# zrjer/Sparse-Matrix-Factorization-Library

Hardware: AMD Instinct MI355X
Metric: numeric-factorization GFLOP/s (supernodal Cholesky) (higher is better)
Workload: dtype f64; 1 GPU; 3D 7-point Laplacian 128^3 SPD Cholesky fp64, geometric ND, devSlotSize 8694792192; n=2097152, nnz_input=8339456, nsuper=35419, factor_doubles=3787034536, parallelism=single GPU, grid_rule=BASELINE config

## Files before the change

sparse-matrix-factorization-library_amd/csrc/sf_kernels.hip:

```cpp
#include "sf_kernels.h"
#include <cstdlib>
#include "sf_wave.h"

namespace sf {

typedef double double4_t __attribute__((ext_vector_type(4)));
typedef double double2_t __attribute__((ext_vector_type(2), aligned(8)));

__device__ __forceinline__ int lower_bound_i32(const int32_t* __restrict__ a, int n, int32_t key) {
    int lo = 0, hi = n;
    while (lo < hi) {
        const int mid = (lo + hi) >> 1;
        if (a[mid] < key) lo = mid + 1; else hi = mid;
    }
    return lo;
}

__global__ void __launch_bounds__(256)
k_load_panels(const int64_t* __restrict__ Lp, const int32_t* __restrict__ Li, const double* __restrict__ Lx, int32_t n,
              const int32_t* __restrict__ Super, const int32_t* __restrict__ SuperMap,
              const int64_t* __restrict__ Lsip, const int32_t* __restrict__ Lsi,
              const int64_t* __restrict__ Lsxp, double* __restrict__ Lsx, int skip_diag,
              const int8_t* __restrict__ load_mask) {
    const int32_t j = blockIdx.x * blockDim.x + threadIdx.x;
// ... 137 lines not shown
    return __hiloint2double(__builtin_amdgcn_readlane(__double2hiint(v), l), __builtin_amdgcn_readlane(__double2loint(v), l));
}

template <bool RCP, int W>
__device__ __forceinline__ void getrf_panel_wave(double (&a)[W], int lane, int J0, int b, double tol, double eps, bool& bad, int& nperturbed,
                                                 int& pos, bool& active, int* piv_rows) {
#pragma unroll
    for (int j = 0; j < W; ++j) {
        const int J = J0 + j;
        int p = J;
        if (tol > 0.0 && J < b) {
            const double nat = readlane_dyn_f64(a[j], J);
            const unsigned long long act = __ballot(active);
            const bool nat_free = ((act >> J) & 1ull) != 0;
            const double anat = fabs(nat);
            const unsigned long long larger = __ballot(active && !(tol * fabs(a[j]) <= anat));
            if (!(nat_free && larger == 0ull && nat != 0.0)) {
                double m;
                const int pm = wave_argmax_abs(a[j], active, &m);
                if (!(nat_free && fabs(nat) >= tol * m && nat != 0.0) && pm >= 0) p = pm;
            }
            p = __builtin_amdgcn_readfirstlane(p);
        }
        double piv = readlane_dyn_f64(a[j], p);
        if (J < b && eps > 0.0 && !(fabs(piv) >= eps) && piv == piv) {
            piv = (piv < 0.0) ? -eps : eps;
            ++nperturbed;
            if (lane == p) a[j] = piv;
        }
        bad = bad || !(piv != 0.0);
        const bool elim = active && lane != p;
        double l;
        if (RCP) {
            const double rp = rcp_full(piv);
            l = elim ? a[j] * rp : 0.0;
        } else {
            l = elim ? a[j] / piv : 0.0;
        }
        if (elim) a[j] = l;
        if (lane == p) { pos = J; active = false; }
        if (piv_rows != nullptr && lane == 0) piv_rows[J] = p;
#pragma unroll
        for (int c = j + 1; c < W; ++c) a[c] -= l * readlane_dyn_f64(a[c], p);
    }
}

template <int W>
__device__ __forceinline__ bool getrf_panel_natural(double (&a)[W], int lane, int J0, int b, double tol, double eps) {
    unsigned long long viol = 0ull;
#pragma unroll
    for (int j = 0; j < W; ++j) {
        const int J = J0 + j;
        const double piv = readlane_dyn_f64(a[j], J);
        const bool below = lane > J;
        viol |= __ballot(below && !(tol * fabs(a[j]) <= fabs(piv)));
        if (J < b && (!(fabs(piv) >= eps) || piv == 0.0)) viol |= 1ull;
        const double rp = rcp_full(piv);
        const double l = below ? a[j] * rp : 0.0;
        if (below) a[j] = l;
#pragma unroll
        for (int c = j + 1; c < W; ++c) a[c] -= l * readlane_dyn_f64(a[c], J);
    }
    return viol == 0ull;
}

template <int W>
__device__ __forceinline__ void getrf_block_w(const PotrfTask& t, double* __restrict__ Lsx, int64_t u_shift, int* __restrict__ info, const PivotCtl& pc) {
    double* PLd = Lsx + t.panel + t.diag + (int64_t)t.diag * t.ld;
    double* PUd = PLd + u_shift;
    const int b = t.b;
    const int lane = threadIdx.x;
    const int64_t ld = t.ld;

    double a[W];
#pragma unroll
    for (int c = 0; c < W; ++c) {
        double v = (c == lane) ? 1.0 : 0.0;
        if (lane < b && c < b) v = (c < lane) ? PLd[lane + c * ld] : PUd[c + lane * ld];
        a[c] = v;
    }
    bool bad = false, active = lane < b;
    int np = 0, pos = lane;
    getrf_panel_wave<false, W>(a, lane, 0, b, pc.tol, pc.eps, bad, np, pos, active, nullptr);
    if (bad && lane == 0) atomicOr(info, 1);
    if (np > 0 && lane == 0) atomicAdd(pc.nperturb, np);
#pragma unroll
    for (int c = 0; c < W; ++c) {
        if (lane < b && c < b) {
            if (c < pos) PLd[pos + c * ld] = a[c]; else PUd[c + pos * ld] = a[c];
        }
    }
    if (pc.pivpos && lane < b) {
        const int g0 = t.first_col + t.diag;
        pc.pivpos[g0 + lane] = g0 + pos;
        pc.pivinv[g0 + pos] = g0 + lane;
    }
}

__global__ void __launch_bounds__(64)
k_getrf_block(const PotrfTask* __restrict__ tasks, double* __restrict__ Lsx, int64_t u_shift, int* __restrict__ info, PivotCtl pc) {
    const PotrfTask t = tasks[blockIdx.x];
    if (t.b <= 8) getrf_block_w<8>(t, Lsx, u_shift, info, pc);
    else if (t.b <= 16) getrf_block_w<16>(t, Lsx, u_shift, info, pc);
    else if (t.b <= 32) getrf_block_w<32>(t, Lsx, u_shift, info, pc);
    else getrf_block_w<NB>(t, Lsx, u_shift, info, pc);
}

void launch_getrf(const PotrfTask* tasks, int ntasks, double* Lsx, int64_t u_shift, int* info, PivotCtl pc, hipStream_t st) {
    if (ntasks <= 0) return;
    hipLaunchKernelGGL(k_getrf_block, dim3(ntasks), dim3(64), 0, st, tasks, Lsx, u_shift, info, pc);
}

__global__ void __launch_bounds__(256)
k_pack_lu(const int32_t* __restrict__ Super, const int64_t* __restrict__ Lsip, const int64_t* __restrict__ Xp,
          const int64_t* __restrict__ RefXp, int32_t nsuper, const double* __restrict__ PL, const double* __restrict__ PU,
          double* __restrict__ out, int64_t e_begin, int64_t e_end) {
    for (int64_t e = e_begin + (int64_t)blockIdx.x * blockDim.x + threadIdx.x; e < e_end; e += (int64_t)gridDim.x * blockDim.x) {
        double* __restrict__ dst = out + (e - e_begin);
        int lo = 0, hi = nsuper;
        while (hi - lo > 1) {
            const int mid = (lo + hi) >> 1;
            if (RefXp[mid] <= e) lo = mid; else hi = mid;
        }
        const int s = lo;
        if (Xp[s] < 0) { *dst = 0.0; continue; }
        const int64_t nscol = Super[s + 1] - Super[s], nsrow = Lsip[s + 1] - Lsip[s];
        const int64_t lda = 2 * nsrow - nscol;
        const int64_t off = e - RefXp[s];
        const int64_t j = off / lda, R = off % lda;
        const double* pl = PL + Xp[s] + j * nsrow;
        double v;
        if (R < nscol) v = (R > j) ? pl[R] : PU[Xp[s] + j + R * nsrow];
        else if (R < nsrow) v = pl[R];
        else v = PU[Xp[s] + (R - nsrow + nscol) + j * nsrow];
        *dst = v;
    }
}

void launch_pack_lu(const int32_t* Super, const int64_t* Lsip, const int64_t* Xp, const int64_t* RefXp, int32_t nsuper,
                    const double* PL, const double* PU, double* out, int64_t e_begin, int64_t e_end, hipStream_t st) {
    if (e_end <= e_begin) return;
    const int64_t blocks = (e_end - e_begin + 255) / 256;
    hipLaunchKernelGGL(k_pack_lu, dim3((unsigned)(blocks < 65536 ? blocks : 65536)), dim3(256), 0, st,
                       Super, Lsip, Xp, RefXp, nsuper, PL, PU, out, e_begin, e_end);
}

__global__ void __launch_bounds__(256)
k_factor_hash(const int32_t* __restrict__ Super, const int64_t* __restrict__ Lsip, const int64_t* __restrict__ Xp,
              const int64_t* __restrict__ RefXp, int32_t nsuper, const double* __restrict__ PL, const double* __restrict__ PU, int lu,
              int64_t total, int64_t chunk, unsigned long long* __restrict__ H) {
    const int64_t begin = (int64_t)blockIdx.x * chunk, end = min(begin + chunk, total);
    if (begin >= end) return;
    const bool idle = begin + threadIdx.x >= end;
    int64_t e = idle ? end - 1 : begin + threadIdx.x;
    int lo = 0, hi = nsuper;
    while (hi - lo > 1) {
        const int mid = (lo + hi) >> 1;
        if (RefXp[mid] <= e) lo = mid; else hi = mid;
    }
    int s = lo;
    unsigned long long acc = 0;
    int64_t s_end = RefXp[s + 1], s_beg = RefXp[s], xp = Xp[s];
    int64_t nscol = Super[s + 1] - Super[s], nsrow = Lsip[s + 1] - Lsip[s];
    if (idle) e = end;
    for (; e < end; e += 256) {
        if (e >= s_end) {
            if (acc) atomicAdd(&H[s], acc);
            acc = 0;
            while (e >= RefXp[s + 1]) ++s;
            s_end = RefXp[s + 1]; s_beg = RefXp[s]; xp = Xp[s];
            nscol = Super[s + 1] - Super[s]; nsrow = Lsip[s + 1] - Lsip[s];
        }
        if (xp < 0) {
            e += ((s_end - e + 255) / 256 - 1) * 256;
            continue;
        }
        const int64_t off = e - s_beg;
        double v;
        if (!lu) {
            v = PL[xp + off];
        } else {
            const int64_t lda = 2 * nsrow - nscol;
            const int64_t j = off / lda, R = off % lda;
            if (R < nscol) v = (R > j) ? PL[xp + j * nsrow + R] : PU[xp + j + R * nsrow];
            else if (R < nsrow) v = PL[xp + j * nsrow + R];
            else v = PU[xp + (R - nsrow + nscol) + j * nsrow];
        }
        acc += (unsigned long long)__double_as_longlong(v) * ((2ull * (unsigned long long)e + 1ull) * 0x9E3779B97F4A7C15ull);
    }
    __shared__ int s_first;
    __shared__ unsigned long long s_part[4];
    if (threadIdx.x == 0) s_first = s;
    __syncthreads();
    const bool uniform = __syncthreads_and(s == s_first) != 0;
    if (!uniform) { if (acc) atomicAdd(&H[s], acc); return; }
    for (int off = 32; off > 0; off >>= 1) acc += __shfl_down(acc, off, 64);
    if ((threadIdx.x & 63) == 0) s_part[threadIdx.x >> 6] = acc;
    __syncthreads();
    if (threadIdx.x == 0) {
        const unsigned long long tot = s_part[0] + s_part[1] + s_part[2] + s_part[3];
        if (tot) atomicAdd(&H[s], tot);
    }
}

void launch_factor_hash(const int32_t* Super, const int64_t* Lsip, const int64_t* Xp, const int64_t* RefXp, int32_t nsuper,
                        const double* PL, const double* PU, int lu, int64_t total, unsigned long long* H, hipStream_t st) {
    if (total <= 0 || nsuper <= 0) return;
    const int64_t chunk = 256 * 64;
    const int64_t blocks = (total + chunk - 1) / chunk;
    hipLaunchKernelGGL(k_factor_hash, dim3((unsigned)blocks), dim3(256), 0, st, Super, Lsip, Xp, RefXp, nsuper, PL, PU, lu, total, chunk, H);
}

__global__ void __launch_bounds__(256)
k_lu_fill_u11(const FillTile* __restrict__ tiles, double* __restrict__ PL, const double* __restrict__ PU) {
    __shared__ double tile[64][65];
    const FillTile t = tiles[blockIdx.x];
    const int tx = threadIdx.x & 63, ty = threadIdx.x >> 6;
    const int jlo = max(t.c0, t.cb), jhi = min(t.c0 + 64, t.ce);
    {
        const int j = t.c0 + tx;
        for (int rr = ty; rr < 64; rr += 4) {
            const int R = t.r0 + rr;
            if (j >= jlo && j < jhi && R <= j) tile[rr][tx] = PU[t.xp + j + (int64_t)R * t.nsrow];
        }
    }
    __syncthreads();
    {
        const int R = t.r0 + tx;
        for (int jj = ty; jj < 64; jj += 4) {
            const int j = t.c0 + jj;
            if (j >= jlo && j < jhi && R <= j) PL[t.xp + R + (int64_t)j * t.nsrow] = tile[tx][jj];
        }
    }
}

void launch_lu_fill_u11(const FillTile* tiles, int64_t ntiles, double* PL, const double* PU, hipStream_t st) {
    if (ntiles <= 0) return;
    hipLaunchKernelGGL(k_lu_fill_u11, dim3((unsigned)ntiles), dim3(256), 0, st, tiles, PL, PU);
}

__global__ void __launch_bounds__(TRSM_ROWS)
k_trsm_block(const TrsmTask* __restrict__ tasks, double* __restrict__ Lsx, const int32_t* __restrict__ pivinv) {
    __shared__ __attribute__((aligned(16))) double Dt[NB][NB];
    __shared__ double Dinv[NB];
    const TrsmTask t = tasks[blockIdx.x];
    const double* Dg = Lsx + t.dpanel + t.diag + (int64_t)t.diag * t.ld;
    const int b = t.b;
    const int tid = threadIdx.x;

    for (int e = tid; e < b * NB; e += (int)blockDim.x) {
        const int k = e / NB, j = e % NB;
        Dt[k][j] = (j < b && k < j) ? Dg[j + (int64_t)k * t.ld] : 0.0;
    }
    if (tid < NB) Dinv[tid] = (tid < b && !t.unit) ? 1.0 / Dg[tid + (int64_t)tid * t.ld] : 1.0;
    __syncthreads();

    if (tid >= t.nrows) return;
    double* X = Lsx + t.panel + t.row0 + tid + (int64_t)t.diag * t.ld;
    const int64_t ld = t.ld;
    if (pivinv && t.unit) {
        const int g0 = t.first_col + t.diag;
        const int32_t* pv = pivinv + g0;
        double tmp[NB];
#pragma unroll
        for (int c = 0; c < NB; ++c) tmp[c] = X[(int64_t)(pv[min(c, b - 1)] - g0) * ld];
#pragma unroll
        for (int c = 0; c < NB; ++c)
            if (c < b) X[(int64_t)c * ld] = tmp[c];
    }

    for (int jb = 0; jb < b; jb += 8) {
        double acc[8];
#pragma unroll
        for (int u = 0; u < 8; ++u) acc[u] = X[min(jb + u, b - 1) * ld];
#pragma unroll
        for (int u = 0; u < 8; ++u) acc[u] = (jb + u < b) ? acc[u] : 0.0;
        for (int k0 = 0; k0 < jb; k0 += 8) {
            double xk[8];
#pragma unroll
            for (int v = 0; v < 8; ++v) xk[v] = X[(k0 + v) * ld];
#pragma unroll
            for (int v = 0; v < 8; ++v)
#pragma unroll
                for (int u = 0; u < 8; ++u) acc[u] -= xk[v] * Dt[k0 + v][jb + u];
        }
#pragma unroll
        for (int u = 0; u < 8; ++u) {
#pragma unroll
            for (int v = 0; v < u; ++v) acc[u] -= acc[v] * Dt[jb + v][jb + u];
            acc[u] *= Dinv[jb + u];
        }
#pragma unroll
        for (int u = 0; u < 8; ++u)
            if (jb + u < b) X[(jb + u) * ld] = acc[u];
    }
}

void launch_trsm(const TrsmTask* tasks, int ntasks, double* Lsx, const int32_t* pivinv, hipStream_t st) {
    if (ntasks <= 0) return;
    hipLaunchKernelGGL(k_trsm_block, dim3(ntasks), dim3(TRSM_ROWS), 0, st, tasks, Lsx, pivinv);
}

constexpr int LDS_LD = GEMM_BM + 16;

__device__ __forceinline__ int last_le_u32(const uint32_t* __restrict__ a, int n, uint32_t key) {
    int lo = 0, hi = n;
    while (hi - lo > 1) {
        const int mid = (lo + hi) >> 1;
        if (a[mid] <= key) lo = mid; else hi = mid;
    }
    return lo;
}

__device__ double g_zero_page[GEMM_BM + 16];

__device__ __forceinline__ void glds16(const void* gsrc, uint32_t lds_dst) {
    unsigned keep;
    asm volatile("s_mov_b32 %0, m0\n\ts_mov_b32 m0, %2\n\ts_nop 0\n\tglobal_load_lds_dwordx4 %1, off\n\ts_mov_b32 m0, %0"
                 : "=&s"(keep) : "v"(gsrc), "s"(lds_dst) : "memory");
}
__device__ __forceinline__ uint32_t lds_addr(const void* p) {
    return __builtin_amdgcn_readfirstlane((uint32_t)(uintptr_t)(__attribute__((address_space(3))) const void*)p);
}

#ifdef SF_EXP_TIMING
__device__ unsigned long long* g_exp_stamps = nullptr;
void exp_set_stamps(unsigned long long* p) { (void)hipMemcpyToSymbol(HIP_SYMBOL(g_exp_stamps), &p, sizeof(p)); }
#define SF_STAMP(slot) do { if (tid == 0 && g_exp_stamps && exp_tile < 64) \
        g_exp_stamps[((size_t)blockIdx.x * 64 + exp_tile) * 4 + (slot)] = __builtin_amdgcn_s_memtime(); } while (0)
#else
#define SF_STAMP(slot) do { } while (0)
#endif

template <int MODE, bool DMA>
__global__ void __launch_bounds__(GEMM_THREADS, GEMM_WAVES / 2)
k_gemm(const GemmProb* __restrict__ probs, const GemmTask* __restrict__ tasks,
       const uint32_t* __restrict__ kt_prefix, int ntasks, uint32_t u_lo, uint32_t u_hi,
       double* __restrict__ Lsx, const int32_t* __restrict__ RelMap, int* __restrict__ ticket, int whole_tiles, uint32_t min_units) {
    __shared__ int s_claim;
    __shared__ __attribute__((aligned(16))) double Ys[2][GEMM_BK][LDS_LD];
    __shared__ __attribute__((aligned(16))) double Xs[2][GEMM_BK][LDS_LD];
    __shared__ int32_t rowmap[GEMM_BM];
    __shared__ int32_t colmap[GEMM_BN];

    constexpr int WCJ = GEMM_BN / (GEMM_WAVES / 2);
    constexpr int TMN = WCJ / 16;
    constexpr int SQ = GEMM_BK / GEMM_WAVES;
    const int tid = threadIdx.x;
    const int lane = tid & 63, wave = tid >> 6;
    const int wm = wave & 1, wn = wave >> 1;
    const int fr = lane & 15, fk = lane >> 4;

    const uint32_t T = u_hi - u_lo;
    const uint32_t G = gridDim.x;
    const uint32_t xcd = blockIdx.x & 7;
    const uint32_t xcd_n = (G >> 3) + (xcd < (G & 7) ? 1u : 0u);
    const uint32_t xcd_base = xcd < (G & 7) ? xcd * ((G >> 3) + 1) : (G & 7) * ((G >> 3) + 1) + (xcd - (G & 7)) * (G >> 3);
    const uint32_t share = xcd_base + (blockIdx.x >> 3);
    (void)T;
    int t0 = last_le_u32(kt_prefix, ntasks + 1, u_lo);
    if (kt_prefix[t0] < u_lo) ++t0;
    const int t1 = last_le_u32(kt_prefix, ntasks + 1, u_hi);
    const int R = (t1 > t0) ? (int)(((uint32_t)(t1 - t0) + (whole_tiles ? G - 1 : 0)) / G) : 0;
    const uint32_t head_end = (R > 0) ? kt_prefix[t0] : u_hi;
    const uint32_t tail_beg = (R > 0 && !whole_tiles) ? kt_prefix[t0 + R * (int)G] : u_hi;

    int ph = 0, rr = 0;
#ifdef SF_EXP_DEPHASE
    bool exp_dephased = false;
#endif
#ifdef SF_EXP_TIMING
    int exp_tile = 0;
    if (tid == 0 && g_exp_stamps) {
        g_exp_stamps[(size_t)gridDim.x * 256 + blockIdx.x * 4 + 0] = __builtin_amdgcn_s_memtime();
        g_exp_stamps[(size_t)gridDim.x * 256 + blockIdx.x * 4 + 1] = wall_clock64();
    }
#endif
    for (;;) {
    uint32_t u, u_end;
    int ti;
    SF_STAMP(0);
    if (ph == 1) {
        uint32_t slot = share;
        if (ticket != nullptr && R > 0) {
            if (tid == 0) s_claim = __hip_atomic_fetch_add(ticket + xcd, 1, __ATOMIC_RELAXED, __HIP_MEMORY_SCOPE_AGENT);
            __syncthreads();
            const uint32_t c = (uint32_t)__builtin_amdgcn_readfirstlane(s_claim);
            rr = (int)(c / xcd_n);
            slot = xcd_base + c % xcd_n;
        }
        if (rr >= R) { ph = 2; continue; }
        ti = t0 + rr * (int)G + (int)slot;
        ++rr;
        if (ti >= t1) continue;
        u = kt_prefix[ti];
        u_end = kt_prefix[ti + 1];
#ifdef SF_EXP_DEPHASE
        if (!exp_dephased && blockIdx.x >= gridDim.x / 2) {
            const int naps = (int)(u_end - u) * SF_EXP_DEPHASE / 16;
            for (int i = 0; i < naps; ++i) __builtin_amdgcn_s_sleep(127);
        }
        exp_dephased = true;
#endif
    } else {
        const uint32_t ra = (ph == 0) ? u_lo : tail_beg, rb = (ph == 0) ? head_end : u_hi;
        const uint32_t Ueq = (rb > ra) ? (rb - ra + G - 1) / G : 0, U = max(Ueq, min_units);
        const uint32_t sh = (U > Ueq) ? blockIdx.x : share;
        if (rb <= ra || sh * U >= rb - ra) {
            if (ph == 0) { ph = 1; continue; }
            break;
        }
        u = ra + sh * U;
        u_end = min(rb, u + U);
        ti = last_le_u32(kt_prefix, ntasks + 1, u);
    }

    while (u < u_end) {
        const GemmTask tk = tasks[ti];
        const GemmProb pb = probs[tk.prob];
        const uint32_t tbase = kt_prefix[ti];
        const int nkt = (int)(kt_prefix[ti + 1] - tbase);
        const int kt0 = (int)(u - tbase);
        const int kt1 = min(nkt, kt0 + (int)(u_end - u));
        u += (uint32_t)(kt1 - kt0);
        ++ti;

        const int ci0 = tk.tm * GEMM_BM, cj0 = tk.tn * GEMM_BN;
        const int M = pb.M, N = pb.N;
        const int lda = pb.lda;
        const int kfirst = (int)tk.kt0 * GEMM_BK;
        const int K = min(pb.K - kfirst, nkt * GEMM_BK);
        const double* __restrict__ Yg = Lsx + pb.y_off + ci0 + (int64_t)kfirst * lda;
        const double* __restrict__ Xg = Lsx + pb.x_off + cj0 + (int64_t)kfirst * lda;

        if (MODE == 1) {
            if (tid < GEMM_BM) {
                const int ci = ci0 + tid;
                rowmap[tid] = (ci < M) ? RelMap[pb.map_off + ci] : 0;
            } else if (tid < GEMM_BM + GEMM_BN) {
                const int cj = cj0 + (tid - GEMM_BM);
                colmap[tid - GEMM_BM] = (cj < N) ? RelMap[pb.map_off + cj] : 0;
            }
        }

        const int prow = 2 * (tid & 63), pk0 = tid >> 6;
        const bool y0_ok = (ci0 + prow) < M, y1_ok = (ci0 + prow + 1) < M;
        const bool x0_ok = (cj0 + prow) < N, x1_ok = (cj0 + prow + 1) < N;
        const double* __restrict__ yp = Yg + (y0_ok ? prow : 0);
        const double* __restrict__ xp = Xg + (x0_ok ? prow : 0);
        double2_t ry[DMA ? 1 : SQ], rx[DMA ? 1 : SQ];

        auto load_tile = [&](int k0) {
            if (DMA) return;
#pragma unroll
            for (int q = 0; q < SQ; ++q) {
                const int64_t off = (int64_t)min(k0 + pk0 + GEMM_WAVES * q, K - 1) * lda;
                ry[q] = *reinterpret_cast<const double2_t*>(yp + off);
                rx[q] = *reinterpret_cast<const double2_t*>(xp + off);
            }
        };
        auto store_tile = [&](int buf, int k0) {
            if (DMA) {
#pragma unroll
                for (int q = 0; q < SQ; ++q) {
                    const int kl = pk0 + GEMM_WAVES * q, k = k0 + kl;
                    const bool kin = k < K;
                    const double* ysrc = yp + (int64_t)min(k, K - 1) * lda;
                    const double* xsrc = kin ? xp + (int64_t)k * lda : g_zero_page + prow;
                    glds16(ysrc, lds_addr(&Ys[buf][kl][0]));
                    glds16(xsrc, lds_addr(&Xs[buf][kl][0]));
                }
                return;
            }
#pragma unroll
            for (int q = 0; q < SQ; ++q) {
                const bool kin = (k0 + pk0 + GEMM_WAVES * q) < K;
                double2_t vy = ry[q], vx = rx[q];
                vy.x = (kin && y0_ok) ? vy.x : 0.0; vy.y = (kin && y1_ok) ? vy.y : 0.0;
                vx.x = (kin && x0_ok) ? vx.x : 0.0; vx.y = (kin && x1_ok) ? vx.y : 0.0;
                *reinterpret_cast<double2_t*>(&Ys[buf][pk0 + GEMM_WAVES * q][prow]) = vy;
                *reinterpret_cast<double2_t*>(&Xs[buf][pk0 + GEMM_WAVES * q][prow]) = vx;
            }
        };

        const int qci0 = ci0 + wm * 64, qcj0 = cj0 + wn * WCJ;
        const bool quad_active = __builtin_amdgcn_readfirstlane((int)((qci0 < M) && (qcj0 < N) && (qci0 + 63 >= qcj0))) != 0;

        double4_t acc[TMN][4];
#pragma unroll
        for (int a = 0; a < TMN; ++a)
#pragma unroll
            for (int b = 0; b < 4; ++b) acc[a][b] = (double4_t){0.0, 0.0, 0.0, 0.0};

        load_tile(kt0 * GEMM_BK);
        store_tile(0, kt0 * GEMM_BK);
        if (DMA) asm volatile("s_waitcnt vmcnt(0)" ::: "memory");
        __syncthreads();
        SF_STAMP(1);
        load_tile((kt0 + 1) * GEMM_BK);
        int buf = 0;
        if (quad_active) {
            for (int kt = kt0; kt < kt1; ++kt) {
#pragma unroll
                for (int kk = 0; kk < GEMM_BK / 4; ++kk) {
                    double a[TMN], b[4];
#pragma unroll
                    for (int t = 0; t < TMN; ++t) a[t] = Xs[buf][kk * 4 + fk][wn * WCJ + t * 16 + fr];
#pragma unroll
                    for (int t = 0; t < 4; ++t) b[t] = Ys[buf][kk * 4 + fk][wm * 64 + t * 16 + fr];
                    if (kk == 0) store_tile(buf ^ 1, (kt + 1) * GEMM_BK);
                    if (kk == 1) load_tile((kt + 2) * GEMM_BK);
#pragma unroll
                    for (int tm = 0; tm < TMN; ++tm)
#pragma unroll
                        for (int tn = 0; tn < 4; ++tn)
                            acc[tm][tn] = __builtin_amdgcn_mfma_f64_16x16x4f64(a[tm], b[tn], acc[tm][tn], 0, 0, 0);
                }
                if (DMA) asm volatile("s_waitcnt vmcnt(0)" ::: "memory");
                __syncthreads();
                buf ^= 1;
            }
        } else {
            for (int kt = kt0; kt < kt1; ++kt) {
                store_tile(buf ^ 1, (kt + 1) * GEMM_BK);
                load_tile((kt + 2) * GEMM_BK);
                if (DMA) asm volatile("s_waitcnt vmcnt(0)" ::: "memory");
                __syncthreads();
                buf ^= 1;
            }
        }

        SF_STAMP(2);
#ifdef SF_EXP_SKIP_EPILOGUE
        if (quad_active) {
            double v = 0.0;
            for (int tm = 0; tm < TMN; ++tm) for (int tn = 0; tn < 4; ++tn) for (int r = 0; r < 4; ++r) v += acc[tm][tn][r];
            if (v == 12345.678) Lsx[pb.c_off] = v;
        }
#else
        if (quad_active) {
            double* __restrict__ Cg = Lsx + pb.c_off;
            const int64_t ldc = pb.ldc;
#pragma unroll
            for (int tm = 0; tm < TMN; ++tm) {
#pragma unroll
                for (int tn = 0; tn < 4; ++tn) {
                    const int lci = wm * 64 + tn * 16 + fr;
                    const int ci = ci0 + lci;
#pragma unroll
                    for (int r = 0; r < 4; ++r) {
                        const int lcj = wn * WCJ + tm * 16 + fk + 4 * r;
                        const int cj = cj0 + lcj;
                        if (ci < M && cj < N && ci >= cj + (pb.strict & 1)) {
                            const double v = acc[tm][tn][r];
                            if (MODE == 1) {
                                unsafeAtomicAdd(Cg + rowmap[lci] + (int64_t)colmap[lcj] * ldc, -v);
                            } else {
                                double* dst = Cg + ci + (int64_t)cj * ldc;
                                unsafeAtomicAdd(dst, -v);
                            }
                        }
                    }
                }
            }
        }
#endif
        __syncthreads();
        SF_STAMP(3);
#ifdef SF_EXP_TIMING
        ++exp_tile;
        SF_STAMP(0);
#endif
    }
    if (ph == 2) break;
    if (ph == 0) ph = 1;
    }
#ifdef SF_EXP_TIMING
    if (tid == 0 && g_exp_stamps) {
        g_exp_stamps[(size_t)gridDim.x * 256 + blockIdx.x * 4 + 2] = __builtin_amdgcn_s_memtime();
        g_exp_stamps[(size_t)gridDim.x * 256 + blockIdx.x * 4 + 3] = wall_clock64();
    }
#endif
}

#ifndef SF_LU_STEP_WGS
#define SF_LU_STEP_WGS 3
#endif
#ifndef SF_GEMM_MIN_UNITS_DEFAULT
#define SF_GEMM_MIN_UNITS_DEFAULT 16
#endif
#ifndef SF_POTRF_PW
#define SF_POTRF_PW 16
#endif
constexpr int ST_ULD = ST_ROWS + 1;
constexpr int ST_KC = 32;
constexpr int ST_XLD = ST_ROWS + 16;
constexpr int ST_SPIN_LIMIT = 1 << 22;

#ifdef SF_EXP_STEP_STAMPS
__device__ unsigned long long* g_step_stamps = nullptr;
void exp_set_step_stamps(unsigned long long* p) { (void)hipMemcpyToSymbol(HIP_SYMBOL(g_step_stamps), &p, sizeof(p)); }
#define ST_STAMP(slot) do { if (is_diag && tid == 0 && g_step_stamps) g_step_stamps[slot] = wall_clock64(); } while (0)
#else
#define ST_STAMP(slot) do { } while (0)
#endif

__device__ __forceinline__ double ld_agent(const double* p) {
    return __hip_atomic_load(p, __ATOMIC_RELAXED, __HIP_MEMORY_SCOPE_AGENT);
}
__device__ __forceinline__ int ld_agent(const int* p) {
    return __hip_atomic_load(p, __ATOMIC_RELAXED, __HIP_MEMORY_SCOPE_AGENT);
}

template <bool LU>
__global__ void __launch_bounds__(256, LU ? SF_LU_STEP_WGS : 3)
k_step(const StepTask* __restrict__ tasks, double* __restrict__ Lsx, int* __restrict__ flags, int epoch, int* __restrict__ info,
       double* __restrict__ tinv, int* __restrict__ ticket, PivotCtl pc) {
    constexpr int SMEM = 2 * ST_KC * ST_XLD;
    __shared__ __attribute__((aligned(16))) double smem[SMEM];
    static_assert(NB == ST_ROWS && NB == 64, "one wavefront per 64 x 64 tile");
    static_assert(NB * ST_ULD <= SMEM && NB * NB + 4 * 256 <= SMEM, "phases must fit the LDS array");
    double* __restrict__ U = smem;
    double (*Dt)[NB] = reinterpret_cast<double (*)[NB]>(smem);

    __shared__ int s_ticket;
    const int tid = threadIdx.x, lane = tid & 63, wave = tid >> 6;
#ifdef SF_EXP_STEP_STAMPS
    const unsigned long long st_entry = wall_clock64();
#endif
    if (tid == 0) s_ticket = __hip_atomic_fetch_add(ticket, 1, __ATOMIC_RELAXED, __HIP_MEMORY_SCOPE_AGENT);
    __syncthreads();
    const StepTask t = tasks[__builtin_amdgcn_readfirstlane(s_ticket)];
    const bool is_pre = LU && (t.mode & 2);
    const bool is_diag = t.row0 == t.diag && !is_pre;
#ifdef SF_EXP_STEP_STAMPS
    if (is_diag && tid == 0 && g_step_stamps) g_step_stamps[0] = st_entry;
#endif
    ST_STAMP(1);
    const int fr = lane & 15, fk = lane >> 4;
    const int64_t ld = t.ld;
    const int b = t.b, nrows = t.nrows;
    const int nhp = ((is_pre ? t.diag - NB : t.diag) - t.J) / NB;
    double* __restrict__ Ag = Lsx + t.panel + t.row0 + (int64_t)t.diag * ld;
    const double* __restrict__ Dg = Lsx + t.xpanel + t.diag + (int64_t)t.diag * ld;

    double4_t acc[4];
#pragma unroll
    for (int a = 0; a < 4; ++a) acc[a] = (double4_t){0.0, 0.0, 0.0, 0.0};

    if (nhp > 0) {
        double (*Xs)[ST_KC][ST_XLD] = reinterpret_cast<double (*)[ST_KC][ST_XLD]>(smem);
        const int nch = 2 * nhp;
        const int prow = 2 * (tid & 31), pk0 = tid >> 5;
        const double* __restrict__ xp = Lsx + t.xpanel + t.diag + (int64_t)t.J * ld + ((prow < b) ? prow : 0);
        const double* __restrict__ yp = Lsx + t.panel + t.row0 + (int64_t)(t.J + fk) * ld + min(16 * wave + fr, nrows - 1);
        const int nhalf = 2 * nch;
        double2_t rx[2][4];
        double fy[4][4];
        auto load_x = [&](int sel, int h) __attribute__((always_inline)) {
            const int hc = min(h, nch - 1);
#pragma unroll
            for (int q = 0; q < 4; ++q) rx[sel][q] = *reinterpret_cast<const double2_t*>(xp + (int64_t)(hc * ST_KC + pk0 + 8 * q) * ld);
        };
        auto store_x = [&](int buf, int sel) __attribute__((always_inline)) {
#pragma unroll
            for (int q = 0; q < 4; ++q) *reinterpret_cast<double2_t*>(&Xs[buf][pk0 + 8 * q][prow]) = rx[sel][q];
        };
        auto load_y = [&](int slot, int hh) __attribute__((always_inline)) {
            const int hc = min(hh, nhalf - 1);
#pragma unroll
            for (int kk = 0; kk < 4; ++kk) fy[slot][kk] = yp[(int64_t)(hc * (ST_KC / 2) + 4 * kk) * ld];
        };
        auto compute = [&](int par, int h) __attribute__((always_inline)) {
            load_y((2 * par + 3) & 3, 2 * h + 3);
#pragma unroll
            for (int kk = 0; kk < 8; ++kk) {
                double a[4];
#pragma unroll
                for (int q = 0; q < 4; ++q) a[q] = Xs[par][4 * kk + fk][16 * q + fr];
                if (kk == 0) store_x(par ^ 1, par ^ 1);
                if (kk == 1) load_x(par ^ 1, h + 3);
                if (kk == 4) load_y(2 * par, 2 * h + 4);
#pragma unroll
                for (int q = 0; q < 4; ++q) acc[q] = __builtin_amdgcn_mfma_f64_16x16x4f64(a[q], fy[2 * par + (kk >> 2)][kk & 3], acc[q], 0, 0, 0);
            }
        };
        load_x(0, 0);
        load_x(1, 1);
        load_y(0, 0);
        load_y(1, 1);
        load_y(2, 2);
        store_x(0, 0);
        load_x(0, 2);
        __syncthreads();
        for (int hp = 0; hp < nhp; ++hp) {
            compute(0, 2 * hp);
            __syncthreads();
            compute(1, 2 * hp + 1);
            __syncthreads();
        }
    }

    if (is_pre) {
        double* __restrict__ Dw = Lsx + t.xpanel + t.diag + (int64_t)t.diag * ld;
        const int ci = 16 * wave + fr;
#pragma unroll
        for (int q = 0; q < 4; ++q)
#pragma unroll
            for (int r = 0; r < 4; ++r) {
                const int cj = 16 * q + fk + 4 * r;
                const int cic = min(ci, b - 1), cjc = min(cj, b - 1);
                const double dl = Ag[cic + (int64_t)cjc * ld], du = Dw[cjc + (int64_t)cic * ld];
                if (ci < b && cj < b) {
                    if (cj < ci) Ag[ci + (int64_t)cj * ld] = dl - acc[q][r];
                    else Dw[cj + (int64_t)ci * ld] = du - acc[q][r];
                }
            }
        return;
    }

    double4_t rt[4];
    if (!is_diag) {
        const int ci = 16 * wave + fr, cic = min(ci, nrows - 1);
#pragma unroll
        for (int q = 0; q < 4; ++q)
#pragma unroll
            for (int r = 0; r < 4; ++r) {
                const int cj = 16 * q + fk + 4 * r;
                const double av = Ag[cic + (int64_t)min(cj, b - 1) * ld];
                rt[q][r] = (ci < nrows && cj < b) ? av - acc[q][r] : 0.0;
            }
    }
    if (LU && is_diag) {
        {
            const int lc = min(lane, b - 1);
            double blk[16];
#pragma unroll
            for (int i = 0; i < 16; ++i) blk[i] = Ag[lc + (int64_t)min(16 * wave + i, b - 1) * ld];
#pragma unroll
            for (int i = 0; i < 16; ++i) {
                const int k = 16 * wave + i;
                if (lane > k) U[k * ST_ULD + lane] = (lane < b && k < b) ? blk[i] : 0.0;
            }
#pragma unroll
            for (int i = 0; i < 16; ++i) blk[i] = Dg[lc + (int64_t)min(16 * wave + i, b - 1) * ld];
#pragma unroll
            for (int i = 0; i < 16; ++i) {
                const int k = 16 * wave + i;
                if (lane >= k) U[lane * ST_ULD + k] = (lane < b && k < b) ? blk[i] : ((lane == k) ? 1.0 : 0.0);
            }
        }
        if (nhp > 0) {
            __syncthreads();
            const int ci = 16 * wave + fr;
#pragma unroll
            for (int q = 0; q < 4; ++q)
#pragma unroll
                for (int r = 0; r < 4; ++r) {
                    const int cj = 16 * q + fk + 4 * r;
                    if (ci < b && cj < b) U[cj * ST_ULD + ci] -= acc[q][r];
                }
        }
    } else if (is_diag) {
        const int ci = 16 * wave + fr;
#pragma unroll
        for (int q = 0; q < 4; ++q)
#pragma unroll
            for (int r = 0; r < 4; ++r) {
                const int cj = 16 * q + fk + 4 * r;
                const int cic = min(ci, nrows - 1), cjc = min(cj, b - 1);
                double v = (ci == cj) ? 1.0 : 0.0;
                const double av = Ag[cic + (int64_t)cjc * ld];
                if (ci < nrows && cj < b && cj <= ci) v = av - acc[q][r];
                U[cj * ST_ULD + ci] = v;
            }
    }

    if (LU && is_diag) {
        __shared__ int s_piv[NB], s_pos[NB];
        if (tid < NB) { s_pos[tid] = -1; s_piv[tid] = tid; }
        __syncthreads();
        ST_STAMP(2);
        bool bad = false, active = lane < b;
        int np = 0, pos = lane;
        bool nat_all = true;
#pragma unroll 1
        for (int q = 0; q < NB / 16; ++q) {
            const int c0 = 16 * q;
            if (wave == 0) {
                double a[16];
#pragma unroll
                for (int u = 0; u < 16; ++u) a[u] = U[(c0 + u) * ST_ULD + lane];
                bool done = false;
                if (nat_all) {
                    done = getrf_panel_natural<16>(a, lane, c0, b, pc.tol, pc.eps);
                    if (done) {
                        if (lane >= c0 && lane < c0 + 16) { active = false; s_piv[lane] = lane; }
                    } else {
#pragma unroll
                        for (int u = 0; u < 16; ++u) a[u] = U[(c0 + u) * ST_ULD + lane];
                    }
                }
                if (!done) {
                    nat_all = false;
                    getrf_panel_wave<true, 16>(a, lane, c0, b, pc.tol, pc.eps, bad, np, pos, active, s_piv);
                }
#pragma unroll
                for (int u = 0; u < 16; ++u) U[(c0 + u) * ST_ULD + lane] = a[u];
                s_pos[lane] = active ? -1 : pos;
            }
            if (q == NB / 16 - 1 || c0 + 16 >= b) break;
            __syncthreads();
            const int ntr = NB - c0 - 16;
            if (tid < ntr) {
                const int c = c0 + 16 + tid;
                double x[16];
                int pr[16];
#pragma unroll
                for (int k = 0; k < 16; ++k) { pr[k] = s_piv[c0 + k]; x[k] = U[c * ST_ULD + pr[k]]; }
#pragma unroll
                for (int k = 1; k < 16; ++k)
#pragma unroll
                    for (int jj = 0; jj < k; ++jj) x[k] -= U[(c0 + jj) * ST_ULD + pr[k]] * x[jj];
#pragma unroll
                for (int k = 1; k < 16; ++k) U[c * ST_ULD + pr[k]] = x[k];
            }
            __syncthreads();
            {
                const int ci = 16 * wave + fr;
                const bool free_row = s_pos[ci] < 0;
                double lf[4];
                int pk[4];
// ... 480 lines not shown
```

Measured before the change: 52730 GFLOP/s.

## Pipeline DMA GEMM loads in half-tile stages with partial vmcnt waits

Restructures the direct-to-LDS (DMA) path of the update GEMM so each K tile is split into two half stages. Each half-stage load is issued while MFMAs run on the other half, and the kernel waits with vmcnt(2) instead of draining all outstanding loads. LDS fragment reads are also double-buffered in registers. The global_load_lds instruction now takes a scalar base plus a per-lane offset, which is meant to save VGPR address computation. In exchange there is one barrier per half tile and a more intricate buffer/phase schedule, which risks races or register pressure.

New measurement: 55980 GFLOP/s (median of 6 runs). 6.2% higher.

```diff
diff --git a/sparse-matrix-factorization-library_amd/csrc/sf_kernels.hip b/sparse-matrix-factorization-library_amd/csrc/sf_kernels.hip
--- a/sparse-matrix-factorization-library_amd/csrc/sf_kernels.hip
+++ b/sparse-matrix-factorization-library_amd/csrc/sf_kernels.hip
@@ -463,6 +463,7 @@
 }
 
 constexpr int LDS_LD = GEMM_BM + 16;
+constexpr int GEMM_SK = GEMM_BK / 2;
 
 __device__ __forceinline__ int last_le_u32(const uint32_t* __restrict__ a, int n, uint32_t key) {
     int lo = 0, hi = n;
@@ -475,10 +476,10 @@
 
 __device__ double g_zero_page[GEMM_BM + 16];
 
-__device__ __forceinline__ void glds16(const void* gsrc, uint32_t lds_dst) {
+__device__ __forceinline__ void glds16(const void* sbase, uint32_t voff, uint32_t lds_dst) {
     unsigned keep;
-    asm volatile("s_mov_b32 %0, m0\n\ts_mov_b32 m0, %2\n\ts_nop 0\n\tglobal_load_lds_dwordx4 %1, off\n\ts_mov_b32 m0, %0"
-                 : "=&s"(keep) : "v"(gsrc), "s"(lds_dst) : "memory");
+    asm volatile("s_mov_b32 %0, m0\n\ts_mov_b32 m0, %3\n\ts_nop 0\n\tglobal_load_lds_dwordx4 %2, %1\n\ts_mov_b32 m0, %0"
+                 : "=&s"(keep) : "s"(sbase), "v"(voff), "s"(lds_dst) : "memory");
 }
 __device__ __forceinline__ uint32_t lds_addr(const void* p) {
     return __builtin_amdgcn_readfirstlane((uint32_t)(uintptr_t)(__attribute__((address_space(3))) const void*)p);
@@ -511,6 +512,8 @@
     const int lane = tid & 63, wave = tid >> 6;
     const int wm = wave & 1, wn = wave >> 1;
     const int fr = lane & 15, fk = lane >> 4;
+    const int swave = __builtin_amdgcn_readfirstlane(wave);
+    const uint32_t lds_ys = lds_addr(&Ys[0][0][0]), lds_xs = lds_addr(&Xs[0][0][0]);
 
     const uint32_t T = u_hi - u_lo;
     const uint32_t G = gridDim.x;
@@ -609,10 +612,10 @@
         const bool x0_ok = (cj0 + prow) < N, x1_ok = (cj0 + prow + 1) < N;
         const double* __restrict__ yp = Yg + (y0_ok ? prow : 0);
         const double* __restrict__ xp = Xg + (x0_ok ? prow : 0);
+        const uint32_t yoff = (y0_ok ? prow : 0) * (uint32_t)sizeof(double), xoff = (x0_ok ? prow : 0) * (uint32_t)sizeof(double);
         double2_t ry[DMA ? 1 : SQ], rx[DMA ? 1 : SQ];
 
         auto load_tile = [&](int k0) {
-            if (DMA) return;
 #pragma unroll
             for (int q = 0; q < SQ; ++q) {
                 const int64_t off = (int64_t)min(k0 + pk0 + GEMM_WAVES * q, K - 1) * lda;
@@ -621,18 +624,6 @@
             }
         };
         auto store_tile = [&](int buf, int k0) {
-            if (DMA) {
-#pragma unroll
-                for (int q = 0; q < SQ; ++q) {
-                    const int kl = pk0 + GEMM_WAVES * q, k = k0 + kl;
-                    const bool kin = k < K;
-                    const double* ysrc = yp + (int64_t)min(k, K - 1) * lda;
-                    const double* xsrc = kin ? xp + (int64_t)k * lda : g_zero_page + prow;
-                    glds16(ysrc, lds_addr(&Ys[buf][kl][0]));
-                    glds16(xsrc, lds_addr(&Xs[buf][kl][0]));
-                }
-                return;
-            }
 #pragma unroll
             for (int q = 0; q < SQ; ++q) {
                 const bool kin = (k0 + pk0 + GEMM_WAVES * q) < K;
@@ -643,6 +634,21 @@
                 *reinterpret_cast<double2_t*>(&Xs[buf][pk0 + GEMM_WAVES * q][prow]) = vx;
             }
         };
+        auto dma_stage = [&](int buf, int half, int kt) {
+            const int kl = half * GEMM_SK + swave, k = kt * GEMM_BK + kl;
+            const uint32_t slot = (uint32_t)((buf * GEMM_BK + kl) * LDS_LD) * (uint32_t)sizeof(double);
+            const bool kin = k < K;
+            const double* ysrc = Yg + (int64_t)min(k, K - 1) * lda;
+            const double* xsrc = kin ? Xg + (int64_t)k * lda : g_zero_page;
+            glds16(ysrc, yoff, lds_ys + slot);
+            glds16(xsrc, xoff, lds_xs + slot);
+        };
+        auto read_frag = [&](double (&a)[TMN], double (&b)[4], int buf, int krow) {
+#pragma unroll
+            for (int t = 0; t < TMN; ++t) a[t] = Xs[buf][krow + fk][wn * WCJ + t * 16 + fr];
+#pragma unroll
+            for (int t = 0; t < 4; ++t) b[t] = Ys[buf][krow + fk][wm * 64 + t * 16 + fr];
+        };
 
         const int qci0 = ci0 + wm * 64, qcj0 = cj0 + wn * WCJ;
         const bool quad_active = __builtin_amdgcn_readfirstlane((int)((qci0 < M) && (qcj0 < N) && (qci0 + 63 >= qcj0))) != 0;
@@ -653,9 +659,66 @@
 #pragma unroll
             for (int b = 0; b < 4; ++b) acc[a][b] = (double4_t){0.0, 0.0, 0.0, 0.0};
 
+        auto mma = [&](const double (&a)[TMN], const double (&b)[4]) {
+#pragma unroll
+            for (int tm = 0; tm < TMN; ++tm)
+#pragma unroll
+                for (int tn = 0; tn < 4; ++tn)
+                    acc[tm][tn] = __builtin_amdgcn_mfma_f64_16x16x4f64(a[tm], b[tn], acc[tm][tn], 0, 0, 0);
+        };
+
+        if constexpr (DMA) {
+        dma_stage(0, 0, kt0);
+        dma_stage(0, 1, kt0);
+        if (kt0 + 1 < kt1) {
+            dma_stage(1, 0, kt0 + 1);
+            asm volatile("s_waitcnt vmcnt(2)" ::: "memory");
+        } else {
+            asm volatile("s_waitcnt vmcnt(0)" ::: "memory");
+        }
+        __syncthreads();
+        SF_STAMP(1);
+        if (quad_active) {
+            double a0[TMN], b0[4], a1[TMN], b1[4];
+            read_frag(a0, b0, 0, 0);
+            auto k_step = [&](const int buf, int kt) {
+#pragma unroll
+                for (int h = 0; h < 2; ++h) {
+                    const bool more = kt + 1 + h < kt1;
+                    read_frag(a1, b1, buf, h * GEMM_SK + 4);
+                    if (more) dma_stage(h ? buf : buf ^ 1, h ^ 1, kt + 1 + h);
+                    mma(a0, b0);
+                    read_frag(a0, b0, h ? buf ^ 1 : buf, h ? 0 : GEMM_SK);
+                    mma(a1, b1);
+                    if (more) asm volatile("s_waitcnt vmcnt(2)" ::: "memory");
+                    else asm volatile("s_waitcnt vmcnt(0)" ::: "memory");
+                    __syncthreads();
+                }
+            };
+            int kt = kt0;
+            for (; kt + 1 < kt1; kt += 2) {
+                k_step(0, kt);
+                k_step(1, kt + 1);
+            }
+            if (kt < kt1) k_step(0, kt);
+        } else {
+            for (int kt = kt0; kt < kt1; ++kt) {
+                const int buf = (kt - kt0) & 1;
+#pragma unroll
+                for (int h = 0; h < 2; ++h) {
+                    if (kt + 1 + h < kt1) {
+                        dma_stage(h ? buf : buf ^ 1, h ^ 1, kt + 1 + h);
+                        asm volatile("s_waitcnt vmcnt(2)" ::: "memory");
+                    } else {
+                        asm volatile("s_waitcnt vmcnt(0)" ::: "memory");
+                    }
+                    __syncthreads();
+                }
+            }
+        }
+        } else {
         load_tile(kt0 * GEMM_BK);
         store_tile(0, kt0 * GEMM_BK);
-        if (DMA) asm volatile("s_waitcnt vmcnt(0)" ::: "memory");
         __syncthreads();
         SF_STAMP(1);
         load_tile((kt0 + 1) * GEMM_BK);
@@ -665,19 +728,11 @@
 #pragma unroll
                 for (int kk = 0; kk < GEMM_BK / 4; ++kk) {
                     double a[TMN], b[4];
-#pragma unroll
-                    for (int t = 0; t < TMN; ++t) a[t] = Xs[buf][kk * 4 + fk][wn * WCJ + t * 16 + fr];
-#pragma unroll
-                    for (int t = 0; t < 4; ++t) b[t] = Ys[buf][kk * 4 + fk][wm * 64 + t * 16 + fr];
+                    read_frag(a, b, buf, kk * 4);
                     if (kk == 0) store_tile(buf ^ 1, (kt + 1) * GEMM_BK);
                     if (kk == 1) load_tile((kt + 2) * GEMM_BK);
-#pragma unroll
-                    for (int tm = 0; tm < TMN; ++tm)
-#pragma unroll
-                        for (int tn = 0; tn < 4; ++tn)
-                            acc[tm][tn] = __builtin_amdgcn_mfma_f64_16x16x4f64(a[tm], b[tn], acc[tm][tn], 0, 0, 0);
+                    mma(a, b);
                 }
-                if (DMA) asm volatile("s_waitcnt vmcnt(0)" ::: "memory");
                 __syncthreads();
                 buf ^= 1;
             }
@@ -685,10 +740,10 @@
             for (int kt = kt0; kt < kt1; ++kt) {
                 store_tile(buf ^ 1, (kt + 1) * GEMM_BK);
                 load_tile((kt + 2) * GEMM_BK);
-                if (DMA) asm volatile("s_waitcnt vmcnt(0)" ::: "memory");
                 __syncthreads();
                 buf ^= 1;
             }
+        }
         }
 
         SF_STAMP(2);
```
